# NVIDIA/KAI-Scheduler

Measured on AMD Instinct MI355X. Metric: pod placements/sec (allocate action, synthetic snapshot), higher is better.
Workload: dtype f64

## Files before the change

kai-scheduler_amd/csrc/kai_fill_levels.hpp:

```cpp
#pragma once
#include "kai_fill_counts.hpp"

namespace kai {

constexpr int KFL_LMAX = 8;
constexpr int KFL_RING = 4096;
constexpr int KFL_XR = 32;
constexpr int KFL_SHORT = 16;
constexpr int KFL_JOB_SHIFT = 23;
constexpr int KFL_PAIRS = KFL_LMAX * (KFL_LMAX - 1) / 2;
constexpr int KFL_WKINDS = 7;
KW_BODY uint64_t kfl_cmd(int g, int g2, int k, int per, int tbase) { return (uint64_t)((uint32_t)g | ((uint32_t)g2 << 4) | ((uint32_t)per << 8) | ((uint32_t)k << 12)) | ((uint64_t)(uint32_t)tbase << 32); }
struct FlMove { uint64_t mask; int32_t w; int32_t seq; };
struct FlLds {
    uint64_t ring[KFL_RING];
    uint64_t dummy[64];
    FlMove x[KFL_PAIRS + 1][KFL_XR];
    FlMove xdummy[64];
    int32_t xtail[KFL_PAIRS];
    int32_t cnt0[KBK_GMAX];
    int32_t tail[KFL_LMAX + 1];
    int32_t head, done, fin, b_dec;
    int64_t w_idle[KFL_LMAX + 1], w_total[KFL_LMAX + 1];
#ifdef KFL_PROF
    int64_t wk_cyc[KFL_LMAX][KFL_WKINDS], wk_cnt[KFL_LMAX][KFL_WKINDS];
#endif
};
#if defined(KFL_PROF) && defined(__HIPCC__)
__device__ int64_t kfl_prof_workers[KFL_LMAX][KFL_WKINDS + 1][2];
#endif
KW_BODY int kfl_pair(int g, int g2) { return (g - 1) * (g - 2) / 2 + (g2 - 1); }
KW_BODY int kfl_div(int a, int b) {
    const uint64_t inv = b <= 4 ? 0x2000'2AAB'4000'8000ull : 0x1000'124A'1556'199Aull;
    return (int)(((uint32_t)a * (uint32_t)((inv >> (16 * ((b - 1) & 3))) & 0xffff)) >> 15);
}
KW_BODY uint64_t kfl_read(KW_LDS_PTR(uint64_t) p) { return kw::bcast(*p, 0); }
KW_BODY void kfl_write(KW_LDS_PTR(uint64_t) p, uint64_t v, KW_LDS_PTR(uint64_t) dummy) { KW_LDS_PTR(uint64_t) q = kw::lane() == 0 ? p : dummy + kw::lane(); *q = v; }
KW_BODY int kfl_load(const int32_t* p) { return kw::uni(kw::lds_load_acq(p)); }
struct FlStretch { int flag, first, nt, q; bool valid, is_def; uint64_t defm, todo; };
KW_BODY uint32_t kfl_tab(int lane, int LV) { uint32_t t = 0; for (int g = 1; g <= LV; g++) t |= (uint32_t)(g / (lane + 1)) << (4 * (g - 1)); return t; }
KW_BODY int kfl_quot(uint32_t tab, int g) { return g >= 1 ? (int)((tab >> (4 * (g - 1))) & 15u) : 0; }
KW_BODY void kfl_classify(FlStretch& s, int ucls, int qk, int capq) {
    int q = kw::shfl(qk, ucls >= 0 ? ucls : 0);
    if (ucls < 0 || q > 31) q = ucls < 0 ? 0 : 31;
    const int cap = kw::shfl(capq, q >= 1 ? q - 1 : 63);
    s.q = q;
    s.is_def = s.valid && s.flag == BF_DEAD && q >= 1 && cap < s.nt;
    s.defm = kw::ballot(s.is_def);
    s.todo = kw::ballot(s.valid && s.flag != BF_GATE && !s.is_def);
}

template <int SP>
KW_BODY void kb_fill_levels_t(const KaiCtx& c, RoundParams rp, BucketParams bp) {
    if (kb_round_off(c.bt)) return;
    KW_SHARED FlLds L;
    const BatchCtx& b = c.bt;
    const int tid = kw::tid(), T = kw::bdim(), lane = kw::lane(), C = c.C;
    BkView v; v.NW = bp.nw; v.NW1 = bp.nw1; v.LV = bp.levels;
    unsigned char* dyn = kw::dyn_lds();
    v.gw = (KW_LDS_PTR(uint64_t))dyn; v.s1 = v.gw + (size_t)v.LV * v.NW; v.ok = v.s1 + (size_t)v.LV * v.NW1 + KBK_GMAX;
    const int64_t tstart = kw::clock();
    if (tid < KBK_GMAX) L.cnt0[tid] = 0;
    if (tid <= KFL_LMAX) { L.tail[tid] = 0; L.w_idle[tid] = 0; L.w_total[tid] = 0; }
    if (tid < KFL_PAIRS) L.xtail[tid] = 0;
#ifdef KFL_PROF
    if (tid < KFL_LMAX * KFL_WKINDS) { L.wk_cyc[tid / KFL_WKINDS][tid % KFL_WKINDS] = 0; L.wk_cnt[tid / KFL_WKINDS][tid % KFL_WKINDS] = 0; }
#endif
    for (int i = tid; i < (KFL_PAIRS + 1) * KFL_XR; i += T) L.x[i / KFL_XR][i % KFL_XR].seq = 0;
    if (tid == 0) { L.head = 0; L.done = 0; L.fin = 0; L.b_dec = 0; }
    for (int i = tid; i < v.LV * v.NW; i += T) v.gw[i] = b.bk_words[i];
    kw::sync();
    for (int i = tid; i < v.LV * v.NW1; i += T) {
        const int l = i / v.NW1, w1 = i % v.NW1; uint64_t m = 0; int pop = 0;
        for (int j = 0; j < 64 && w1 * 64 + j < v.NW; j++) { const uint64_t x = v.gw[l * v.NW + w1 * 64 + j]; if (x) { m |= 1ull << j; pop += __builtin_popcountll(x); } }
        v.s1[i] = m;
        if (pop) kw::atomic_add((int32_t*)&L.cnt0[l], pop);
    }
    kw::sync();
    const int V = rp.mode != 1 ? b.q_valid[c.Q] : 0;
    const int wave = kw::uni(tid >> 6);
    if (wave == 0) {
#ifdef KFL_PRIO
        kw::set_prio<KFL_PRIO>();
#endif
        int cnt = lane < v.LV ? L.cnt0[lane] : 0;
        const bool act = lane < C;
        const int qk = act ? (int)c.cls[lane].req[KAI_RES_GPU] : 0x7fffffff;
        const uint32_t tab = kfl_tab(lane, v.LV);
        const int invq = (int)(((lane < 4 ? 0x2000'2AAB'4000'8000ull : 0x1000'124A'1556'199Aull) >> (16 * (lane & 3))) & 0xffff);
        uint32_t nz = (uint32_t)kw::ballot(cnt > 0);
        int decisions = 0, attempted = 0, committed = 0, rollbacks = 0, ops = 0, n_done = rp.start, mismatch = 0;
        int wp = 0, tail_seen = 0, pub = 0, n_mark = 0;
        int64_t a_wait = 0;
#ifdef KFL_PROF
        int64_t pc[5] = {0, 0, 0, 0, 0}; int64_t pt = kw::clock();
        #define KFL_T(i) do { const int64_t n_ = kw::clock(); pc[i] += n_ - pt; pt = n_; } while (0)
#else
        #define KFL_T(i) (void)0
#endif
        auto tails_min = [&]() { int t = lane <= v.LV ? kw::lds_load_acq(&L.tail[lane < v.LV ? lane : KFL_LMAX]) : 0x7fffffff; for (int l = 1; l <= v.LV; l++) { const int o = kw::bcast(t, l); t = o < t ? o : t; } return kw::bcast(t, 0); };
        #define KFL_LEVEL_FOR(qc) ((nz >> ((qc) - 1)) ? (SP ? 32 - __builtin_clz(nz) : (qc) + __builtin_ctz(nz >> ((qc) - 1))) : 0)
        #define KFL_ROOM(n) do { if (wp - tail_seen > KFL_RING - (n)) { kw::lds_store_rel(&L.head, wp); pub = wp; const int64_t w0 = kw::clock(); while (wp - tail_seen > KFL_RING - (n)) { tail_seen = tails_min(); if (wp - tail_seen > KFL_RING - (n)) kw::relax(); } a_wait += kw::clock() - w0; } } while (0)
        #define KFL_EMIT(g_, g2_, k_, per_, tb_) do { KW_LDS_PTR(uint64_t) sl_ = lane == 0 ? (KW_LDS_PTR(uint64_t))&L.ring[wp & (KFL_RING - 1)] : (KW_LDS_PTR(uint64_t))&L.dummy[lane]; *sl_ = kfl_cmd(g_, g2_, k_, per_, tb_) | jbits; wp++; } while (0)
        #define KFL_EVENT(g_, g2_, k_, cg_) do { const int e_g = (g_), e_g2 = (g2_), e_k = (k_), e_cg = (cg_); \
            cnt = kw::writelane(cnt, e_cg - e_k, (e_g - 1) & 63); \
            const uint32_t e_in = e_g2 >= 1 ? 1u << ((e_g2 - 1) & 31) : 0u, e_out = (uint32_t)(e_cg - e_k - 1) >> 31;   \
            cnt = kw::writelane(cnt, kw::bcast(cnt, (e_g2 - 1) & 63) + e_k, (e_g2 - 1) & 63); \
            nz = (nz & ~(e_out << ((e_g - 1) & 31))) | e_in; } while (0)
        #define KFL_STEP(S, EMIT) \
            const uint32_t lv##S = nz >> (qc - 1); \
            ok = kw::nonzero01(lv##S);   \
            const int g##S = lv##S ? (SP ? 32 - __builtin_clz(nz) : qc + __builtin_ctz(lv##S)) : 0, gm1##S = g##S - 1; \
            int r##S = SP ? 1 : (int)((tq >> ((4 * g##S - 4) & 31)) & 15u); r##S = r##S > 1 ? r##S : 1;   \
            const int rem##S = nt - placed; \
            const int kq##S = SP ? rem##S : (int)(((uint32_t)rem##S * (uint32_t)kw::bcast(invq, r##S - 1)) >> 15);   \
            const int cg##S = kw::bcast(cnt, gm1##S & 63); \
            int k##S = kq##S < cg##S ? kq##S : cg##S; k##S = (k##S > 1 ? k##S : 1) * ok;   \
            const int per##S = r##S < rem##S ? r##S : rem##S, g2##S = g##S - per##S * qc; \
            EMIT(g##S, g2##S, k##S, per##S); \
            KFL_EVENT(g##S, g2##S, k##S, cg##S); \
            placed += k##S * per##S
        #define KFL_EMIT_RING(g_, g2_, k_, per_) KFL_EMIT(g_, g2_, k_, per_, first + placed)
        #define KFL_LOW(g_, g2_, k_, per_) (int)((uint32_t)(g_) | ((uint32_t)(g2_) << 4) | ((uint32_t)(per_) << 8) | ((uint32_t)(k_) << 12))
        #define KFL_HOLD0(g_, g2_, k_, per_) c0 = kw::writelane(c0, KFL_LOW(g_, g2_, k_, per_), jj)
        #define KFL_HOLD1(g_, g2_, k_, per_) c1 = kw::writelane(c1, KFL_LOW(g_, g2_, k_, per_), jj)
        #define KFL_GANG_END() \
            okm |= (uint64_t)(uint32_t)(1 - fail) << jj; failm |= (uint64_t)(uint32_t)fail << jj; \
            extra += placed & (0 - fail); \
            cnt = fail ? cnt_s : cnt; nz = fail ? nz_s : nz; wp = fail ? wp_s : wp; \
            const int mism = (int)((uint32_t)(flag - 1) >> 31) ^ fail ^ 1;   \
            mismatch |= mism; last_jj = jj
        int nx_flag = 0, nx_first = 0, nx_nt = 0, nx_ucls = 0;
        if (V > rp.start) { const int gc = rp.start + lane < V ? rp.start + lane : V - 1; nx_flag = b.g_flag[gc]; nx_first = b.g_first[gc]; nx_nt = b.g_nt[gc]; nx_ucls = b.g_ucls[gc]; }
        for (int base = rp.start; base < V && !mismatch; base += 64) {
            const int gi = base + lane;
            FlStretch s; s.valid = gi < V;
            s.flag = s.valid ? nx_flag : (int)BF_GATE; s.first = s.valid ? nx_first : 0; s.nt = s.valid ? nx_nt : 0;
            const int my_ucls = s.valid ? nx_ucls : 0;
            { const int gc = gi + 64 < V ? gi + 64 : V - 1; nx_flag = b.g_flag[gc]; nx_first = b.g_first[gc]; nx_nt = b.g_nt[gc]; nx_ucls = b.g_ucls[gc]; }
            const int jn = V - base < 64 ? V - base : 64;
            int capq = 0;
            for (int g = 1; g <= v.LV; g++) capq += kfl_quot(tab, g) * kw::bcast(cnt, g - 1);
            kfl_classify(s, my_ucls, qk, capq);
            const int my_pack = s.flag | (s.q << 2) | (s.nt << 7) | ((s.q == 0 || s.nt > KFL_SHORT || s.nt < 1) ? 1 << 18 : 0) | (s.flag == BF_OK ? 1 << 19 : 0);
            const uint32_t my_tq = kw::shfl(tab, s.q >= 1 ? s.q - 1 : 63);
            uint64_t longm = kw::ballot(((my_pack >> 18) & 1) != 0);
            uint64_t todo = s.todo, okm = 0, failm = 0, okw = 0;
            int n_out = jn, last_jj = 0, extra = 0;
            attempted += jn; n_done = base + jn;
            KFL_ROOM(1);
#if defined(__HIP_DEVICE_COMPILE__)
            asm volatile("s_waitcnt lgkmcnt(0)" :: "v"(my_tq), "v"(my_pack) : "memory");
#endif
            { KW_LDS_PTR(uint64_t) sl_ = lane == 0 ? (KW_LDS_PTR(uint64_t))&L.ring[wp & (KFL_RING - 1)] : (KW_LDS_PTR(uint64_t))&L.dummy[lane]; *sl_ = 0; wp++; n_mark++; }
            KFL_T(0);
            while (todo) {
                const uint64_t lm = todo & longm;
                const uint64_t below = lm ? (lm & (0 - lm)) - 1 : ~0ull;
                uint64_t hot = todo & below;
                todo &= ~below;
                if (hot) {
                    const uint64_t run0 = hot; uint64_t twor = 0, rest = 0;
                    int c0 = 0, c1 = 0, jj, pred, ok;
                    do {
                        jj = __builtin_ctzll(hot); hot &= hot - 1;
                        const int pack = kw::bcast(my_pack, jj);
                        const uint32_t tq = kw::bcast(my_tq, jj);
                        const int qc = (pack >> 2) & 31, nt = (pack >> 7) & 0x7ff;
                        pred = (pack >> 19) & 1;
                        KFL_T(1);
                        const uint32_t nz_s = nz;
                        int placed = 0;
                        KFL_STEP(A, KFL_HOLD0);
                        if (__builtin_expect(placed < nt * ok, 0)) {
                            int cnt_s = kw::writelane(cnt, kw::bcast(cnt, (g2A - 1) & 63) - kA, (g2A - 1) & 63); cnt_s = kw::writelane(cnt_s, cgA, gm1A & 63);
                            KFL_STEP(B, KFL_HOLD1);
                            if (!ok) { cnt = cnt_s; nz = nz_s; extra += placed; }
                            else if (placed < nt) {
                                cnt = cnt_s; nz = nz_s; longm |= 1ull << jj; rest = hot | (1ull << jj); hot = 0; ok = pred;
                            } else twor |= 1ull << jj;
                        }
                        KFL_T(2);
                        okw |= (uint64_t)(uint32_t)ok << jj;
                        hot = kw::opaque(pred == ok ? hot : (uint64_t)0);
                        KFL_T(3);
                    } while (hot);
                    mismatch |= pred ^ ok;
                    const uint64_t walked = run0 & ((2ull << jj) - 1) & ~rest, okr = walked & okw;
                    failm |= walked & ~okw; hot |= rest;
                    okm |= okr;
                    if (mismatch) last_jj = 63 - __builtin_clzll(walked);
                    if (okr) {
                        const int n_my = (int)((okr >> lane) & 1ull) + (int)((twor >> lane) & 1ull);
                        const int incl = kw::wave_scan_add(n_my), n_run = kw::bcast(incl, 63);
                        KFL_ROOM(n_run);
                        const int pos = wp + incl - n_my;
                        const uint32_t jb = (uint32_t)lane << KFL_JOB_SHIFT;
                        if (n_my >= 1) L.ring[pos & (KFL_RING - 1)] = (uint64_t)((uint32_t)c0 | jb) | ((uint64_t)(uint32_t)s.first << 32);
                        if (n_my >= 2) L.ring[(pos + 1) & (KFL_RING - 1)] = (uint64_t)((uint32_t)c1 | jb) | ((uint64_t)(uint32_t)(s.first + ((c0 >> 12) & 0x7ff) * ((c0 >> 8) & 15)) << 32);
                        wp += n_run;
                        kw::lds_store_rel(&L.head, wp); pub = wp;
                    }
                    KFL_T(3);
                }
                todo |= hot;
                if (mismatch) break;
                if (!hot && lm) {
                    const int jj = __builtin_ctzll(todo); todo &= todo - 1;
                    const int pack = kw::bcast(my_pack, jj), first = kw::bcast(s.first, jj);
                    const uint32_t tq = kw::bcast(my_tq, jj);
                    const int flag = pack & 3, qc = (pack >> 2) & 31, nt = (pack >> 7) & 0x7ff;
                    const uint64_t jbits = (uint64_t)((uint32_t)jj << KFL_JOB_SHIFT);
                    KFL_T(1);
                    const int cnt_s = cnt, wp_s = wp; const uint32_t nz_s = nz;
                    int placed = 0, ok = 1;
                    KFL_ROOM(nt);
                    if (!qc) {
                        for (int tb = 0; tb < nt && ok; tb += 64) {
                            const int my_cls = tb + lane < nt ? b.t_cls[first + tb + lane] : 0;
                            const int tc = nt - tb < 64 ? nt - tb : 64;
                            for (int ti = 0; ti < tc; ti++) {
                                const int q1 = kw::bcast(qk, kw::bcast(my_cls, ti));
                                const int g = q1 <= 31 ? KFL_LEVEL_FOR(q1) : 0;
                                if (!g) { ok = 0; break; }
                                KFL_EMIT(g, g - q1, 1, 1, first + placed);
                                KFL_EVENT(g, g - q1, 1, kw::bcast(cnt, g - 1));
                                placed++;
                            }
                        }
                    } else while ((placed < nt) & (ok != 0)) { KFL_STEP(L, KFL_EMIT_RING); }
                    const int fail = ok ^ 1;
                    KFL_T(2);
                    KFL_GANG_END();
                    if (wp - pub >= 64) { kw::lds_store_rel(&L.head, wp); pub = wp; }
                    KFL_T(3);
                    if (mism) break;
                }
            }
            if (mismatch) { n_done = base + last_jj + 1; n_out = last_jj + 1; attempted -= jn - n_out; }
            KFL_T(3);
            {
                const uint64_t outm = n_out >= 64 ? ~0ull : (1ull << n_out) - 1;
                const int nfail = __builtin_popcountll(s.defm & outm) + __builtin_popcountll(failm);
                decisions += nfail + extra; rollbacks += 2 * nfail;
                const bool my_ok = (okm >> lane) & 1ull;
                const int myv = my_ok ? s.nt : 0, incl = kw::wave_scan_add(myv);
                const int my_stmt = committed + rp.stmt0 + __builtin_popcountll(okm & ((1ull << lane) - 1)), my_opoff = ops + rp.ops0 + incl - myv;
                if (lane < n_out) { b.g_out[base + lane] = (uint8_t)(my_ok ? BF_OK : BF_DEAD); b.g_opoff[base + lane] = my_opoff; b.g_stmt[base + lane] = my_stmt; }
                committed += __builtin_popcountll(okm); ops += kw::bcast(incl, 63); decisions += kw::bcast(incl, 63);
            }
            if (wp != pub) { kw::lds_store_rel(&L.head, wp); pub = wp; }
            KFL_T(4);
        }
        #undef KFL_LEVEL_FOR
        #undef KFL_ROOM
        #undef KFL_EMIT
        #undef KFL_EVENT
        #undef KFL_STEP
        #undef KFL_EMIT_RING
        #undef KFL_LOW
        #undef KFL_HOLD0
        #undef KFL_HOLD1
        #undef KFL_GANG_END
        if (lane == 0) L.fin = n_done;
        kw::lds_store_rel(&L.head, wp);
        kw::lds_store_rel(&L.done, 1);
        const uint64_t dead = kw::ballot(act && (qk > 32 || (nz >> (qk - 1)) == 0));
        if (lane == 0) {
            FillStatus s; s.n_done = n_done; s.mismatch = mismatch; s.all_dead = (C > 0 && dead == (C >= 64 ? ~0ull : ((1ull << C) - 1))) ? 1 : 0; s.planned = V; s.floor_stop = 0; s.pad = 0;
            s.decisions = decisions; s.attempted = attempted; s.committed = committed; s.rollbacks = rollbacks; s.ops = ops; s.dead_mask = dead;
            s.cycles_total = kw::clock() - tstart; s.cycles_load = a_wait; s.cycles_update = 0; s.cycles_rescan = 0; s.block_loads = 0;
            s.rescans1 = 0; s.rescans2 = wp - n_mark; s.rescans3 = 0;
#ifdef KFL_PROF
            s.cycles_load = pc[0]; s.cycles_update = pc[1]; s.cycles_rescan = pc[2]; s.block_loads = pc[3]; s.rescans1 = pc[4];
#endif
            b.fs[0] = s; b.dead_mask[0] = dead;
        }
    } else if (wave <= v.LV) {
        const int G = wave, lw = (G - 1) * v.NW, l1 = (G - 1) * v.NW1;
        KW_LDS_PTR(uint64_t) dm = (KW_LDS_PTR(uint64_t))&L.dummy[0];
        uint64_t s1v = lane < v.NW1 ? v.s1[l1 + lane] : 0;
        uint64_t s2 = kw::ballot(s1v != 0);
        int firstn = KB_INF, cw = -1; uint64_t curw = 0;
        auto refill = [&]() { if (!s2) { firstn = KB_INF; cw = -1; curw = 0; return; } const int w1 = __builtin_ctzll(s2); cw = w1 * 64 + __builtin_ctzll(kw::bcast(s1v, w1)); curw = kfl_read(&v.gw[lw + cw]); firstn = (cw << 6) + __builtin_ctzll(curw); };
        refill();
        int xp = 0, xseen = 0, xc = 0;
        int tail = 0; int64_t w_idle = 0; const int64_t w_start = kw::clock();
#ifdef KFL_PROF
        int64_t wt = kw::clock();
        #define KFL_WT0() (wt = kw::clock())
        #define KFL_WK(kind_) do { const int64_t n_ = kw::clock(); if (lane == 0) { L.wk_cyc[G - 1][kind_] += n_ - wt; L.wk_cnt[G - 1][kind_]++; } wt = n_; } while (0)
#else
        #define KFL_WT0() (void)0
        #define KFL_WK(kind_) (void)0
#endif
        for (;;) {
            const int head = kfl_load(&L.head);
            if (tail == head) {
                if (kfl_load(&L.done) && tail == kfl_load(&L.head)) break;
                const int64_t i0 = kw::clock(); while (kfl_load(&L.head) == tail && !kfl_load(&L.done)) kw::relax(); w_idle += kw::clock() - i0;
                continue;
            }
            while (tail < head) {
                const int nb = head - tail < 64 ? head - tail : 64;
                const uint64_t mc = L.ring[(tail + lane) & (KFL_RING - 1)];
                uint64_t mine = kw::ballot(lane < nb && ((int)(mc & 15) == G || (int)((mc >> 4) & 15) == G));
                while (mine) {
                    KFL_WT0();
                    const int ci = __builtin_ctzll(mine); mine &= mine - 1;
                    const int ca = kw::bcast((int)(uint32_t)mc, ci);
                    const int g = ca & 15, g2 = (ca >> 4) & 15;
                    if (g == G) {
                        const int per = (ca >> 8) & 15; int left = (ca >> 12) & 0x7ff, tb = kw::bcast((int)(uint32_t)(mc >> 32), ci);
                        const int pr = g2 >= 1 ? kfl_pair(G, g2) : KFL_PAIRS;
                        const int xl = (g2 - 1) & 63;
#ifdef KFL_PROF
                        const int k_all = left; int n_words = 0, n_emptied = 0;
#endif
                        if (__builtin_expect(left == 1, 1)) {
                            const int w = cw; const uint64_t mask = curw & (0 - curw), neww = curw ^ mask;
                            b.t_node[tb + (lane < per ? lane : per - 1)] = firstn;
                            kfl_write(&v.gw[lw + w], neww, dm);
                            const int n_w = kw::bcast(xp, xl);
                            if (__builtin_expect(n_w - kw::bcast(xseen, xl) >= KFL_XR, 0)) { int t; while (n_w - (t = kfl_load(&L.xtail[pr])) >= KFL_XR) kw::relax(); if (lane == xl) xseen = t; }
                            KW_LDS_PTR(FlMove) e = lane == 0 ? (KW_LDS_PTR(FlMove))&L.x[pr][n_w & (KFL_XR - 1)] : (KW_LDS_PTR(FlMove))&L.xdummy[lane];
                            e->mask = mask; e->w = w | (1 << 30);
                            kw::lds_store_ordered((int32_t*)&e->seq, n_w + 1);
                            xp += lane == g2 - 1 ? 1 : 0;
                            if (__builtin_expect(neww != 0, 1)) { curw = neww; firstn = (w << 6) + __builtin_ctzll(neww); }
                            else {
                                const int w1 = w >> 6; const uint64_t m1 = kw::bcast(s1v, w1) & ~(1ull << (w & 63));
                                s1v = kw::writelane(s1v, m1, w1);
                                s2 &= ~((uint64_t)(uint32_t)(1 - kw::nonzero01((uint32_t)m1 | (uint32_t)(m1 >> 32))) << w1);
                                refill();
#ifdef KFL_PROF
                                n_emptied++;
#endif
                            }
                            left = 0;
                        }
                        while (__builtin_expect(left > 0, 0)) {
                            const int w = cw; const uint64_t word = curw;
                            const int pop = __builtin_popcountll(word), m = left < pop ? left : pop;
                            const int r = kw::rank_below(word);
                            const bool sel = ((word >> lane) & 1ull) != 0 && r < m;
                            const uint64_t mask = kw::ballot(sel), neww = word ^ mask;
                            const int one = m == 1, lastn = (w << 6) + 63 - __builtin_clzll(mask);
                            const int val = sel ? (w << 6) + lane : lastn;
                            const int onem = 0 - one, off1 = lane < per ? lane : per - 1, offm = sel ? r * per : m * per - 1;
                            int a = tb + ((off1 & onem) | (offm & ~onem));
                            b.t_node[a] = val;
                            if (__builtin_expect((per & ~onem) > 1, 0)) {
                                const int stp = sel ? 1 : 0;
                                _Pragma("nounroll") for (int j = 1; j < per; j++) { a += stp; b.t_node[a] = val; }
                            }
                            kfl_write(&v.gw[lw + w], neww, dm);
                            left -= m; tb += m * per;
                            const int n_w = kw::bcast(xp, xl);
                            if (__builtin_expect(n_w - kw::bcast(xseen, xl) >= KFL_XR, 0)) { int t; while (n_w - (t = kfl_load(&L.xtail[pr])) >= KFL_XR) kw::relax(); if (lane == xl) xseen = t; }
                            KW_LDS_PTR(FlMove) e = lane == 0 ? (KW_LDS_PTR(FlMove))&L.x[pr][n_w & (KFL_XR - 1)] : (KW_LDS_PTR(FlMove))&L.xdummy[lane];
                            e->mask = mask; e->w = w | (left == 0 ? 1 << 30 : 0);
                            kw::lds_store_ordered((int32_t*)&e->seq, n_w + 1);
                            xp += lane == g2 - 1 ? 1 : 0;
                            if (__builtin_expect(neww != 0, 1)) { curw = neww; firstn = (w << 6) + __builtin_ctzll(neww); }
                            else {
                                const int w1 = w >> 6; const uint64_t m1 = kw::bcast(s1v, w1) & ~(1ull << (w & 63));
                                s1v = kw::writelane(s1v, m1, w1);
                                s2 &= ~((uint64_t)(uint32_t)(1 - kw::nonzero01((uint32_t)m1 | (uint32_t)(m1 >> 32))) << w1);
                                refill();
#ifdef KFL_PROF
                                n_emptied++;
#endif
                            }
#ifdef KFL_PROF
                            n_words++;
#endif
                        }
#ifdef KFL_PROF
                        if (k_all == 1) { if (n_emptied) KFL_WK(1); else KFL_WK(0); } else if (n_words == 1) KFL_WK(2); else KFL_WK(3);
#endif
                    } else {
                        const int pr = kfl_pair(g, G);
                        for (bool last = false; !last;) {
                            const int n_r = kw::bcast(xc, g - 1);
                            const int sl = n_r & (KFL_XR - 1);
                            int sq = kw::lds_load_ordered(&L.x[pr][sl].seq), wf_v = kw::lds_load_relaxed(&L.x[pr][sl].w); uint64_t mk_v = kw::lds_load_relaxed(&L.x[pr][sl].mask);
                            if (__builtin_expect(kw::uni(sq) != n_r + 1, 0)) { const int64_t i0 = kw::clock(); while (kfl_load(&L.x[pr][sl].seq) != n_r + 1) kw::relax(); w_idle += kw::clock() - i0; wf_v = kw::lds_load_relaxed(&L.x[pr][sl].w); mk_v = kw::lds_load_relaxed(&L.x[pr][sl].mask); KFL_WT0(); }
                            const int wf = kw::bcast(wf_v, 0), w = wf & 0x3fffffff; const uint64_t mask = kw::bcast(mk_v, 0);
                            last = (wf >> 30) & 1;
                            kw::lds_store_ordered(&L.xtail[pr], n_r + 1);
                            if (lane == g - 1) xc++;
                            if (w == cw) { curw |= mask; kfl_write(&v.gw[lw + w], curw, dm); firstn = (w << 6) + __builtin_ctzll(curw); KFL_WK(4); }
                            else {
                                const int w1 = w >> 6;
#ifdef KFL_PROF
                                const bool was_empty = ((kw::bcast(s1v, w1) >> (w & 63)) & 1ull) == 0;
#endif
                                { KW_LDS_PTR(uint64_t) q = lane == 0 ? (KW_LDS_PTR(uint64_t))&v.gw[lw + w] : dm + lane; kw::lds_or(q, mask); }
                                s1v = kw::writelane(s1v, kw::bcast(s1v, w1) | (1ull << (w & 63)), w1); s2 |= 1ull << w1;
                                const int n = (w << 6) + __builtin_ctzll(mask), fn = kw::uni(firstn);
                                const bool lower = n < fn;
                                firstn = lower ? n : fn; cw = lower ? w : cw; curw = lower ? mask : curw;
#ifdef KFL_PROF
                                if (was_empty) KFL_WK(5); else KFL_WK(6);
#endif
                            }
                        }
                    }
                }
                tail += nb;
            }
            kw::lds_store_rel(&L.tail[G - 1], tail);
        }
        #undef KFL_WT0
        #undef KFL_WK
        if (lane == 0) { L.w_idle[G - 1] = w_idle; L.w_total[G - 1] = kw::clock() - w_start; }
    } else if (wave == v.LV + 1) {
        const int qk = lane < C ? (int)c.cls[lane].req[KAI_RES_GPU] : 0x7fffffff;
        const uint32_t tab = kfl_tab(lane, v.LV);
        int capq = 0;
// ... 70 lines not shown
```

kai-scheduler_amd/csrc/kai_simt.hpp:

```cpp
#pragma once
#include <stdint.h>

#if defined(__HIPCC__)
#include <hip/hip_runtime.h>

#include "kai_wave.hpp"
#define KW_DEV __device__ __forceinline__
#define KW_BODY __device__ __forceinline__
#define KW_SHARED __shared__
#define KW_LDS_PTR(T) T __attribute__((address_space(3)))*
namespace kw {
KW_DEV int tid() { return (int)threadIdx.x; }
KW_DEV int bid() { return (int)blockIdx.x; }
KW_DEV int bdim() { return (int)blockDim.x; }
KW_DEV int gdim() { return (int)gridDim.x; }
KW_DEV int lane() { return (int)(threadIdx.x & 63); }
KW_DEV void sync() { __syncthreads(); }
KW_DEV uint64_t ballot(bool p) { return (uint64_t)__ballot(p); }
template <class T> KW_DEV T shfl(T v, int src) { return __shfl(v, src, 64); }
KW_DEV uint64_t shfl(uint64_t v, int src) { return (uint64_t)__shfl((unsigned long long)v, src, 64); }
KW_DEV int64_t shfl(int64_t v, int src) { return (int64_t)__shfl((long long)v, src, 64); }
template <class T> KW_DEV T shfl_up(T v, int d) { return __shfl_up(v, d, 64); }
KW_DEV uint64_t wave_max_u64(uint64_t v) { return (uint64_t)kai::wave_max_u64((unsigned long long)v); }
KW_DEV int bcast(int v, int src) { return __builtin_amdgcn_readlane(v, __builtin_amdgcn_readfirstlane(src)); }
KW_DEV uint32_t bcast(uint32_t v, int src) { return (uint32_t)bcast((int)v, src); }
KW_DEV uint64_t bcast(uint64_t v, int src) { const int s = __builtin_amdgcn_readfirstlane(src); return ((uint64_t)(uint32_t)__builtin_amdgcn_readlane((int)(v >> 32), s) << 32) | (uint32_t)__builtin_amdgcn_readlane((int)v, s); }
KW_DEV double bcast(double v, int src) { return __longlong_as_double((long long)bcast((uint64_t)__double_as_longlong(v), src)); }
KW_DEV int uni(int v) { return __builtin_amdgcn_readfirstlane(v); }
KW_DEV uint32_t uni(uint32_t v) { return (uint32_t)__builtin_amdgcn_readfirstlane((int)v); }
KW_DEV uint64_t uni(uint64_t v) { return ((uint64_t)(uint32_t)__builtin_amdgcn_readfirstlane((int)(v >> 32)) << 32) | (uint32_t)__builtin_amdgcn_readfirstlane((int)v); }
extern "C" __device__ int kw_llvm_writelane(int v, int dst, int old) __asm("llvm.amdgcn.writelane.i32");
KW_DEV int writelane(int old, int v, int dst) { return kw_llvm_writelane(__builtin_amdgcn_readfirstlane(v), __builtin_amdgcn_readfirstlane(dst), old); }
KW_DEV uint64_t writelane(uint64_t old, uint64_t v, int dst) { return ((uint64_t)(uint32_t)writelane((int)(old >> 32), (int)(v >> 32), dst) << 32) | (uint32_t)writelane((int)old, (int)v, dst); }
KW_DEV int rank_below(uint64_t m) { return (int)__builtin_amdgcn_mbcnt_hi((uint32_t)(m >> 32), __builtin_amdgcn_mbcnt_lo((uint32_t)m, 0u)); }
KW_DEV int nonzero01(uint32_t v) { int r; asm("s_min_u32 %0, %1, 1" : "=s"(r) : "s"(v) : "scc"); return r; }
KW_DEV uint64_t opaque(uint64_t v) { v = uni(v); asm("" : "+s"(v)); return v; }
template <int P> KW_DEV void set_prio() { __builtin_amdgcn_s_setprio(P); }
KW_DEV int atomic_add(int32_t* p, int v) { return atomicAdd(p, v); }
KW_DEV int atomic_min(int32_t* p, int v) { return atomicMin(p, v); }
KW_DEV int atomic_max(int32_t* p, int v) { return atomicMax(p, v); }
KW_DEV unsigned long long atomic_add(unsigned long long* p, unsigned long long v) { return atomicAdd(p, v); }
KW_DEV unsigned long long atomic_or(unsigned long long* p, unsigned long long v) { return atomicOr(p, v); }
KW_DEV double atomic_add(double* p, double v) { return atomicAdd(p, v); }
KW_DEV uint32_t atomic_or32(uint32_t* p, uint32_t v) { return atomicOr(p, v); }
KW_DEV int64_t clock() { return (int64_t)clock64(); }
KW_DEV unsigned char* dyn_lds() { extern __shared__ __align__(16) unsigned char kw_dyn_lds_[]; return kw_dyn_lds_; }
KW_DEV void fence() { __threadfence(); }
KW_DEV void wave_sync() { __builtin_amdgcn_fence(__ATOMIC_RELEASE, "workgroup"); __builtin_amdgcn_wave_barrier(); __builtin_amdgcn_fence(__ATOMIC_ACQUIRE, "workgroup"); }
KW_DEV void lds_order() { __builtin_amdgcn_fence(__ATOMIC_RELEASE, "wavefront"); __builtin_amdgcn_wave_barrier(); __builtin_amdgcn_fence(__ATOMIC_ACQUIRE, "wavefront"); }
KW_DEV uint64_t lds_xor(KW_LDS_PTR(uint64_t) p, uint64_t v) { return __hip_atomic_fetch_xor(p, v, __ATOMIC_RELAXED, __HIP_MEMORY_SCOPE_WAVEFRONT); }
KW_DEV void lds_or(KW_LDS_PTR(uint64_t) p, uint64_t v) { (void)__hip_atomic_fetch_or(p, v, __ATOMIC_RELAXED, __HIP_MEMORY_SCOPE_WAVEFRONT); }
KW_DEV void expect_uniform(long long) {}
KW_DEV void fence_wg() { __builtin_amdgcn_fence(__ATOMIC_RELEASE, "workgroup"); __builtin_amdgcn_fence(__ATOMIC_ACQUIRE, "workgroup"); }
KW_DEV int lds_load_acq(const int32_t* p) { return __hip_atomic_load(p, __ATOMIC_ACQUIRE, __HIP_MEMORY_SCOPE_WORKGROUP); }
KW_DEV void lds_store_rel(int32_t* p, int v) { __hip_atomic_store(p, v, __ATOMIC_RELEASE, __HIP_MEMORY_SCOPE_WORKGROUP); }
KW_DEV void relax() { __builtin_amdgcn_s_sleep(1); }
KW_DEV void lds_store_ordered(int32_t* p, int v) { __builtin_amdgcn_fence(__ATOMIC_RELEASE, "wavefront"); __hip_atomic_store(p, v, __ATOMIC_RELAXED, __HIP_MEMORY_SCOPE_WORKGROUP); }
KW_DEV int lds_load_ordered(const int32_t* p) { const int v = __hip_atomic_load(p, __ATOMIC_RELAXED, __HIP_MEMORY_SCOPE_WORKGROUP); __builtin_amdgcn_fence(__ATOMIC_ACQUIRE, "wavefront"); return v; }
KW_DEV int lds_load_relaxed(const int32_t* p) { return __hip_atomic_load(p, __ATOMIC_RELAXED, __HIP_MEMORY_SCOPE_WORKGROUP); }
KW_DEV uint64_t lds_load_relaxed(const uint64_t* p) { return __hip_atomic_load(p, __ATOMIC_RELAXED, __HIP_MEMORY_SCOPE_WORKGROUP); }
}

#else
#include <cstdio>
#include <cstdlib>
#include <cstring>
#include <functional>
#include <vector>
#define KW_DEV inline
#define KW_BODY inline
#define KW_LDS_PTR(T) T*
#define KW_SHARED static
namespace kw {

extern "C" void kw_switch_ctx(void** save_sp, void* load_sp);
#if defined(__x86_64__)
asm(R"(
.text
.globl kw_switch_ctx
.type kw_switch_ctx,@function
kw_switch_ctx:
    pushq %rbp
    pushq %rbx
    pushq %r12
    pushq %r13
    pushq %r14
    pushq %r15
    movq %rsp, (%rdi)
    movq %rsi, %rsp
    popq %r15
    popq %r14
    popq %r13
    popq %r12
    popq %rbx
    popq %rbp
    ret
.size kw_switch_ctx,.-kw_switch_ctx
)");
#else
#error "the host emulator's context switch is written for x86-64"
#endif

enum FiberState : int { F_RUN = 0, F_WAIT_BLOCK = 1, F_WAIT_WAVE = 2, F_DONE = 3 };
struct Fiber { void* sp = nullptr; int state = F_DONE; char* stack = nullptr; int line = 0; };
struct Emu {
    std::vector<Fiber> fibers; std::vector<char*> stacks;
    void* sched_sp = nullptr;
    int cur = -1, block = 0, bdim = 0, gdim = 0;
    const std::function<void()>* body = nullptr;
    uint64_t xchg[64 * 64];
    std::vector<unsigned char> lds;
    static constexpr size_t STACK = 128 * 1024;
};
inline Emu& emu() { static Emu e; return e; }
inline void fiber_yield() { Emu& e = emu(); kw_switch_ctx(&e.fibers[e.cur].sp, e.sched_sp); }
inline void fiber_entry() {
    Emu& e = emu();
    (*e.body)();
    e.fibers[e.cur].state = F_DONE;
    fiber_yield();
    std::abort();
}
inline void launch(int grid, int block, size_t dyn_lds_bytes, const std::function<void()>& body) {
    Emu& e = emu();
    if (grid <= 0 || block <= 0) return;
    if (block > 64 * 64) { std::fprintf(stderr, "kw::launch: workgroup too large\n"); std::abort(); }
    e.lds.assign(dyn_lds_bytes + 64, 0);
    e.body = &body; e.bdim = block; e.gdim = grid;
    if ((int)e.fibers.size() < block) e.fibers.resize(block);
    while ((int)e.stacks.size() < block) e.stacks.push_back(static_cast<char*>(std::malloc(Emu::STACK)));
    for (int b = 0; b < grid; b++) {
        e.block = b;
        for (int t = 0; t < block; t++) {
            Fiber& f = e.fibers[t]; f.stack = e.stacks[t]; f.state = F_RUN;
            uintptr_t top = (reinterpret_cast<uintptr_t>(f.stack) + Emu::STACK) & ~uintptr_t(15);
            void** sp = reinterpret_cast<void**>(top) - 2;
            *sp = reinterpret_cast<void*>(&fiber_entry);
            for (int i = 0; i < 6; i++) *--sp = nullptr;
            f.sp = sp;
        }
        int live = block;
        static const int order = [] { const char* v = std::getenv("KW_EMU_ORDER"); return v ? std::atoi(v) : 0; }();
        static uint64_t rng = [] { const char* v = std::getenv("KW_EMU_SEED"); return 0x9e3779b97f4a7c15ull + (v ? (uint64_t)std::atoll(v) * 0x100000001b3ull : 0); }();
        while (live > 0) {
            bool progress = false;
            const int nwv = (block + 63) / 64;
            for (int wi = 0; wi < nwv; wi++) {
                const int w = order == 1 ? nwv - 1 - wi : wi;
                if (order == 2) { rng = rng * 6364136223846793005ull + 1442695040888963407ull; if ((rng >> 40) & 1) continue; }
                for (int t = w * 64; t < block && t < w * 64 + 64; t++) {
                    if (e.fibers[t].state != F_RUN) continue;
                    e.cur = t; kw_switch_ctx(&e.sched_sp, e.fibers[t].sp);
                    progress = true;
                    if (e.fibers[t].state == F_DONE) live--;
                }
            }
            if (order == 2 && !progress) { bool any = false; for (int t = 0; t < block; t++) if (e.fibers[t].state == F_RUN) any = true; if (any) continue; }
            bool all_block = true; int waiting = 0;
            for (int t = 0; t < block; t++) { int s = e.fibers[t].state; if (s == F_RUN || s == F_WAIT_WAVE) all_block = false; if (s == F_WAIT_BLOCK) waiting++; }
            if (all_block && waiting) { for (int t = 0; t < block; t++) if (e.fibers[t].state == F_WAIT_BLOCK) e.fibers[t].state = F_RUN; progress = true; }
            for (int w = 0; w * 64 < block; w++) {
                bool all = true; int nw = 0;
                for (int t = w * 64; t < block && t < w * 64 + 64; t++) { int s = e.fibers[t].state; if (s == F_RUN || s == F_WAIT_BLOCK) all = false; if (s == F_WAIT_WAVE) nw++; }
                if (all && nw) { for (int t = w * 64; t < block && t < w * 64 + 64; t++) if (e.fibers[t].state == F_WAIT_WAVE) e.fibers[t].state = F_RUN; progress = true; }
            }
            if (!progress && live > 0) {
                std::fprintf(stderr, "kw::launch: deadlock (a collective not reached by every live lane); block %d, lanes parked at source lines:", b);
                for (int t = 0; t < block && t < 64; t++) std::fprintf(stderr, " %d:%s%d", t, e.fibers[t].state == F_WAIT_BLOCK ? "B" : e.fibers[t].state == F_WAIT_WAVE ? "W" : e.fibers[t].state == F_DONE ? "done" : "run", e.fibers[t].line);
                std::fprintf(stderr, "\n"); std::abort();
            }
        }
    }
    e.body = nullptr;
}
inline int tid() { return emu().cur; }
inline int bid() { return emu().block; }
inline int bdim() { return emu().bdim; }
inline int gdim() { return emu().gdim; }
inline int lane() { return emu().cur & 63; }
inline void sync(int line = __builtin_LINE()) { Emu& e = emu(); e.fibers[e.cur].line = line; e.fibers[e.cur].state = F_WAIT_BLOCK; fiber_yield(); }
inline void wave_bar(int line = 0) { Emu& e = emu(); if (line) e.fibers[e.cur].line = line; e.fibers[e.cur].state = F_WAIT_WAVE; fiber_yield(); }
inline uint64_t* wave_slots() { Emu& e = emu(); return e.xchg + (size_t)(e.cur >> 6) * 64; }
inline bool lane_live(int l) { Emu& e = emu(); int t = (e.cur & ~63) + l; return t < e.bdim && e.fibers[t].state != F_DONE; }
template <class T> inline T shfl(T v, int src, int line = __builtin_LINE()) {
    static_assert(sizeof(T) <= 8, "shfl: 8 bytes at most");
    uint64_t raw = 0; std::memcpy(&raw, &v, sizeof(T));
    wave_slots()[lane()] = raw; wave_bar(line);
    uint64_t got = wave_slots()[src & 63]; wave_bar();
    T r; std::memcpy(&r, &got, sizeof(T)); return r;
}
template <class T> inline T shfl_up(T v, int d) { int l = lane(); T r = shfl(v, l >= d ? l - d : l); return l >= d ? r : v; }
inline uint64_t ballot(bool p, int line = __builtin_LINE()) {
    wave_slots()[lane()] = p ? 1 : 0; wave_bar(line);
    uint64_t m = 0; for (int l = 0; l < 64; l++) if (lane_live(l) && wave_slots()[l]) m |= 1ull << l;
    wave_bar(); return m;
}
inline uint64_t wave_max_u64(uint64_t v, int line = __builtin_LINE()) {
    wave_slots()[lane()] = v; wave_bar(line);
    uint64_t m = 0; for (int l = 0; l < 64; l++) if (lane_live(l) && wave_slots()[l] > m) m = wave_slots()[l];
    wave_bar(); return m;
}
template <class T> inline T bcast(T v, int src, int line = __builtin_LINE()) { return shfl(v, src, line); }
template <class T> inline T uni(T v) { return v; }
inline int writelane(int old, int v, int dst) { return lane() == dst ? v : old; }
inline uint64_t writelane(uint64_t old, uint64_t v, int dst) { return lane() == dst ? v : old; }
inline int rank_below(uint64_t m) { return __builtin_popcountll(m & ((1ull << lane()) - 1)); }
inline int nonzero01(uint32_t v) { return v ? 1 : 0; }
inline uint64_t opaque(uint64_t v) { return v; }
template <int P> inline void set_prio() {}
inline int atomic_add(int32_t* p, int v) { int o = *p; *p = o + v; return o; }
inline int atomic_min(int32_t* p, int v) { int o = *p; if (v < o) *p = v; return o; }
inline int atomic_max(int32_t* p, int v) { int o = *p; if (v > o) *p = v; return o; }
inline unsigned long long atomic_add(unsigned long long* p, unsigned long long v) { unsigned long long o = *p; *p = o + v; return o; }
inline unsigned long long atomic_or(unsigned long long* p, unsigned long long v) { unsigned long long o = *p; *p = o | v; return o; }
inline double atomic_add(double* p, double v) { double o = *p; *p = o + v; return o; }
inline uint32_t atomic_or32(uint32_t* p, uint32_t v) { uint32_t o = *p; *p = o | v; return o; }
inline int64_t clock() { return 0; }
inline unsigned char* dyn_lds() { Emu& e = emu(); return reinterpret_cast<unsigned char*>((reinterpret_cast<uintptr_t>(e.lds.data()) + 15) & ~uintptr_t(15)); }
inline void fence() {}
inline void fence_wg() {}
inline int lds_load_acq(const int32_t* p) { return *p; }
inline void lds_store_rel(int32_t* p, int v) { *p = v; }
inline void lds_store_ordered(int32_t* p, int v) { *p = v; }
inline int lds_load_ordered(const int32_t* p) { return *p; }
inline int lds_load_relaxed(const int32_t* p) { return *p; }
inline uint64_t lds_load_relaxed(const uint64_t* p) { return *p; }
inline void relax(int line = __builtin_LINE()) { wave_bar(line); }
inline void wave_sync(int line = __builtin_LINE()) { wave_bar(line); }
inline void lds_order(int line = __builtin_LINE()) { wave_bar(line); }
inline uint64_t lds_xor(uint64_t* p, uint64_t v) { const uint64_t o = *p; *p = o ^ v; return o; }
inline void lds_or(uint64_t* p, uint64_t v) { *p |= v; }
inline void expect_uniform(long long v, int line = __builtin_LINE()) { const long long v0 = shfl(v, 0, line); if (v != v0) { std::fprintf(stderr, "kw: value not uniform at line %d: lane %d has %lld, lane 0 has %lld\n", line, lane(), v, v0); std::abort(); } }
}
#endif

namespace kw {
KW_DEV void wave_argmax_first(uint64_t& key, int& n) {
    const uint64_t m = wave_max_u64(key);
    const uint64_t win = ballot(key == m);
    const int l = __builtin_ctzll(win);
    n = shfl(n, l);
    key = m;
}
template <class T> KW_DEV T wave_scan_add(T v) {
    for (int d = 1; d < 64; d <<= 1) { T o = shfl_up(v, d); if (lane() >= d) v = v + o; }
    return v;
}
#if defined(__HIPCC__)
#define KW_DPP_MOV(x, ctrl, rmask) __builtin_amdgcn_update_dpp(0, (int)(x), ctrl, rmask, 0xf, false)
template <> KW_DEV int wave_scan_add<int>(int v) {
    v += KW_DPP_MOV(v, 0x111, 0xf); v += KW_DPP_MOV(v, 0x112, 0xf); v += KW_DPP_MOV(v, 0x114, 0xf); v += KW_DPP_MOV(v, 0x118, 0xf);
    v += KW_DPP_MOV(v, 0x142, 0xa); v += KW_DPP_MOV(v, 0x143, 0xc);
    return v;
}
template <int CTRL, int RMASK> KW_DEV int dpp_mov32(int x) { return __builtin_amdgcn_update_dpp(0, x, CTRL, RMASK, 0xf, false); }
template <int CTRL, int RMASK> KW_DEV uint64_t dpp_mov64(uint64_t x) { return ((uint64_t)(unsigned)dpp_mov32<CTRL, RMASK>((int)(x >> 32)) << 32) | (unsigned)dpp_mov32<CTRL, RMASK>((int)x); }
template <> KW_DEV double wave_scan_add<double>(double v) {
#define KW_DPP_ADD_F64(ctrl, rmask) { const long long b_ = __double_as_longlong(v); const unsigned lo_ = (unsigned)KW_DPP_MOV((unsigned)b_, ctrl, rmask), hi_ = (unsigned)KW_DPP_MOV((unsigned)((unsigned long long)b_ >> 32), ctrl, rmask); v = v + __longlong_as_double((long long)(((unsigned long long)hi_ << 32) | lo_)); }
    KW_DPP_ADD_F64(0x111, 0xf) KW_DPP_ADD_F64(0x112, 0xf) KW_DPP_ADD_F64(0x114, 0xf) KW_DPP_ADD_F64(0x118, 0xf) KW_DPP_ADD_F64(0x142, 0xa) KW_DPP_ADD_F64(0x143, 0xc)
#undef KW_DPP_ADD_F64
    return v;
}
#endif
}
```

Before: 8.229 million.

## Precompute per-lane fill decisions in a table and shift level indexing by one

The hot gang-placement loop now uses a per-lane decision word computed in parallel across the wave (KFL_TABLE) while the level bitmap is unchanged. It replaces the serial per-gang KFL_STEP computation with a broadcast and a few scalar ops, and recomputes the table only when the bitmap changes. Level counts are re-indexed from 1 with bit 0 of nz used as a sentinel, so level 0 absorbs gangs that drain a level. Bit updates use scalar s_bitset instructions. This adds complexity and recomputation whenever nz changes, and carries a correctness risk in the reworked mismatch and fail bookkeeping.

```diff
diff --git a/kai-scheduler_amd/csrc/kai_fill_levels.hpp b/kai-scheduler_amd/csrc/kai_fill_levels.hpp
--- a/kai-scheduler_amd/csrc/kai_fill_levels.hpp
+++ b/kai-scheduler_amd/csrc/kai_fill_levels.hpp
@@ -83,12 +83,12 @@
 #ifdef KFL_PRIO
         kw::set_prio<KFL_PRIO>();
 #endif
-        int cnt = lane < v.LV ? L.cnt0[lane] : 0;
+        int cnt = lane >= 1 && lane <= v.LV ? L.cnt0[lane - 1] : 0;
         const bool act = lane < C;
         const int qk = act ? (int)c.cls[lane].req[KAI_RES_GPU] : 0x7fffffff;
         const uint32_t tab = kfl_tab(lane, v.LV);
         const int invq = (int)(((lane < 4 ? 0x2000'2AAB'4000'8000ull : 0x1000'124A'1556'199Aull) >> (16 * (lane & 3))) & 0xffff);
-        uint32_t nz = (uint32_t)kw::ballot(cnt > 0);
+        uint32_t nz = (uint32_t)kw::ballot(cnt > 0) | 1u;
         int decisions = 0, attempted = 0, committed = 0, rollbacks = 0, ops = 0, n_done = rp.start, mismatch = 0;
         int wp = 0, tail_seen = 0, pub = 0, n_mark = 0;
         int64_t a_wait = 0;
@@ -99,22 +99,22 @@
         #define KFL_T(i) (void)0
 #endif
         auto tails_min = [&]() { int t = lane <= v.LV ? kw::lds_load_acq(&L.tail[lane < v.LV ? lane : KFL_LMAX]) : 0x7fffffff; for (int l = 1; l <= v.LV; l++) { const int o = kw::bcast(t, l); t = o < t ? o : t; } return kw::bcast(t, 0); };
-        #define KFL_LEVEL_FOR(qc) ((nz >> ((qc) - 1)) ? (SP ? 32 - __builtin_clz(nz) : (qc) + __builtin_ctz(nz >> ((qc) - 1))) : 0)
+        #define KFL_LEVEL_FOR(qc) (((nz >> 1) >> ((qc) - 1)) ? (SP ? 31 - __builtin_clz(nz) : (qc) + __builtin_ctz((nz >> 1) >> ((qc) - 1))) : 0)
         #define KFL_ROOM(n) do { if (wp - tail_seen > KFL_RING - (n)) { kw::lds_store_rel(&L.head, wp); pub = wp; const int64_t w0 = kw::clock(); while (wp - tail_seen > KFL_RING - (n)) { tail_seen = tails_min(); if (wp - tail_seen > KFL_RING - (n)) kw::relax(); } a_wait += kw::clock() - w0; } } while (0)
         #define KFL_EMIT(g_, g2_, k_, per_, tb_) do { KW_LDS_PTR(uint64_t) sl_ = lane == 0 ? (KW_LDS_PTR(uint64_t))&L.ring[wp & (KFL_RING - 1)] : (KW_LDS_PTR(uint64_t))&L.dummy[lane]; *sl_ = kfl_cmd(g_, g2_, k_, per_, tb_) | jbits; wp++; } while (0)
-        #define KFL_EVENT(g_, g2_, k_, cg_) do { const int e_g = (g_), e_g2 = (g2_), e_k = (k_), e_cg = (cg_); \
-            cnt = kw::writelane(cnt, e_cg - e_k, (e_g - 1) & 63); \
-            const uint32_t e_in = e_g2 >= 1 ? 1u << ((e_g2 - 1) & 31) : 0u, e_out = (uint32_t)(e_cg - e_k - 1) >> 31;   \
-            cnt = kw::writelane(cnt, kw::bcast(cnt, (e_g2 - 1) & 63) + e_k, (e_g2 - 1) & 63); \
-            nz = (nz & ~(e_out << ((e_g - 1) & 31))) | e_in; } while (0)
+        #define KFL_EVENT(g_, g2_, k_, cg_) do { const int e_g = (g_), e_g2 = (g2_) > 0 ? (g2_) : 0, e_k = (k_), e_cg = (cg_); \
+            const int e_t = kw::bcast(cnt, e_g2 & 63); \
+            cnt = kw::writelane(cnt, e_cg - e_k, e_g & 63); \
+            cnt = kw::writelane(cnt, e_t + e_k, e_g2 & 63);   \
+            nz = kw::bit_set(kw::bit_clear(nz, e_cg == e_k ? e_g : 31), e_g2); } while (0)
         #define KFL_STEP(S, EMIT) \
-            const uint32_t lv##S = nz >> (qc - 1); \
+            const uint32_t lv##S = nz >> qc; \
             ok = kw::nonzero01(lv##S);   \
-            const int g##S = lv##S ? (SP ? 32 - __builtin_clz(nz) : qc + __builtin_ctz(lv##S)) : 0, gm1##S = g##S - 1; \
+            const int g##S = lv##S ? (SP ? 31 - __builtin_clz(nz) : qc + __builtin_ctz(lv##S)) : 0; \
             int r##S = SP ? 1 : (int)((tq >> ((4 * g##S - 4) & 31)) & 15u); r##S = r##S > 1 ? r##S : 1;   \
             const int rem##S = nt - placed; \
             const int kq##S = SP ? rem##S : (int)(((uint32_t)rem##S * (uint32_t)kw::bcast(invq, r##S - 1)) >> 15);   \
-            const int cg##S = kw::bcast(cnt, gm1##S & 63); \
+            const int cg##S = kw::bcast(cnt, g##S & 63); \
             int k##S = kq##S < cg##S ? kq##S : cg##S; k##S = (k##S > 1 ? k##S : 1) * ok;   \
             const int per##S = r##S < rem##S ? r##S : rem##S, g2##S = g##S - per##S * qc; \
             EMIT(g##S, g2##S, k##S, per##S); \
@@ -122,15 +122,26 @@
             placed += k##S * per##S
         #define KFL_EMIT_RING(g_, g2_, k_, per_) KFL_EMIT(g_, g2_, k_, per_, first + placed)
         #define KFL_LOW(g_, g2_, k_, per_) (int)((uint32_t)(g_) | ((uint32_t)(g2_) << 4) | ((uint32_t)(per_) << 8) | ((uint32_t)(k_) << 12))
-        #define KFL_HOLD0(g_, g2_, k_, per_) c0 = kw::writelane(c0, KFL_LOW(g_, g2_, k_, per_), jj)
         #define KFL_HOLD1(g_, g2_, k_, per_) c1 = kw::writelane(c1, KFL_LOW(g_, g2_, k_, per_), jj)
+        #define KFL_TABLE() do { \
+            const int t_q = s.q >= 1 ? s.q : 1, t_nt = s.nt; \
+            const uint32_t t_lv = nz >> t_q; \
+            const int t_g = SP ? 31 - __builtin_clz(nz) : t_q + __builtin_ctz(t_lv | 0x80000000u); \
+            int t_r = SP ? 1 : (int)((my_tq >> ((4 * t_g - 4) & 31)) & 15u); t_r = t_r > 1 ? t_r : 1; \
+            const int t_kq = SP ? t_nt : kfl_div(t_nt, t_r), t_kq1 = t_kq > 1 ? t_kq : 1; \
+            const int t_per = t_r < t_nt ? t_r : t_nt, t_g2 = t_g - t_per * t_q; \
+            const uint32_t t_p = s.flag == BF_OK ? 1u : 0u; \
+            const uint32_t t_w = (uint32_t)t_g | ((uint32_t)t_g2 << 4) | ((uint32_t)t_per << 8) | ((uint32_t)t_kq1 << 23) | (t_kq1 * t_per < t_nt ? 1u << 28 : 0u) | (1u << 29) | ((t_p ^ 1u) << 30); \
+            dw = t_lv ? t_w : t_p << 30; nz_tab = nz; mism = kw::ballot(((dw >> 30) & 1u) != 0); } while (0)
+        #define KFL_CUT(h) do { const uint64_t c_m = (h) & mism, c_keep = c_m ? ((c_m & (0 - c_m)) << 1) - 1 : ~0ull; held = (h) & ~c_keep; (h) &= c_keep; } while (0)
         #define KFL_GANG_END() \
             okm |= (uint64_t)(uint32_t)(1 - fail) << jj; failm |= (uint64_t)(uint32_t)fail << jj; \
             extra += placed & (0 - fail); \
             cnt = fail ? cnt_s : cnt; nz = fail ? nz_s : nz; wp = fail ? wp_s : wp; \
-            const int mism = (int)((uint32_t)(flag - 1) >> 31) ^ fail ^ 1;   \
-            mismatch |= mism; last_jj = jj
+            const int g_mis = (int)((uint32_t)(flag - 1) >> 31) ^ fail ^ 1;   \
+            mismatch |= g_mis; last_jj = jj
         int nx_flag = 0, nx_first = 0, nx_nt = 0, nx_ucls = 0;
+        uint32_t dw = 0, nz_tab = ~0u; uint64_t mism = 0;
         if (V > rp.start) { const int gc = rp.start + lane < V ? rp.start + lane : V - 1; nx_flag = b.g_flag[gc]; nx_first = b.g_first[gc]; nx_nt = b.g_nt[gc]; nx_ucls = b.g_ucls[gc]; }
         for (int base = rp.start; base < V && !mismatch; base += 64) {
             const int gi = base + lane;
@@ -140,12 +151,13 @@
             { const int gc = gi + 64 < V ? gi + 64 : V - 1; nx_flag = b.g_flag[gc]; nx_first = b.g_first[gc]; nx_nt = b.g_nt[gc]; nx_ucls = b.g_ucls[gc]; }
             const int jn = V - base < 64 ? V - base : 64;
             int capq = 0;
-            for (int g = 1; g <= v.LV; g++) capq += kfl_quot(tab, g) * kw::bcast(cnt, g - 1);
+            for (int g = 1; g <= v.LV; g++) capq += kfl_quot(tab, g) * kw::bcast(cnt, g);
             kfl_classify(s, my_ucls, qk, capq);
             const int my_pack = s.flag | (s.q << 2) | (s.nt << 7) | ((s.q == 0 || s.nt > KFL_SHORT || s.nt < 1) ? 1 << 18 : 0) | (s.flag == BF_OK ? 1 << 19 : 0);
             const uint32_t my_tq = kw::shfl(tab, s.q >= 1 ? s.q - 1 : 63);
             uint64_t longm = kw::ballot(((my_pack >> 18) & 1) != 0);
-            uint64_t todo = s.todo, okm = 0, failm = 0, okw = 0;
+            nz_tab = ~0u;
+            uint64_t todo = s.todo, okm = 0, failm = 0;
             int n_out = jn, last_jj = 0, extra = 0;
             attempted += jn; n_done = base + jn;
             KFL_ROOM(1);
@@ -160,32 +172,46 @@
                 uint64_t hot = todo & below;
                 todo &= ~below;
                 if (hot) {
-                    const uint64_t run0 = hot; uint64_t twor = 0, rest = 0;
-                    int c0 = 0, c1 = 0, jj, pred, ok;
+                    const uint64_t run0 = hot; uint64_t twor = 0, rest = 0, fail2 = 0, held;
+                    int c0 = 0, c1 = 0, jj; uint32_t w;
+                    if (nz != nz_tab) { KFL_TABLE(); }
+                    KFL_CUT(hot);
                     do {
-                        jj = __builtin_ctzll(hot); hot &= hot - 1;
-                        const int pack = kw::bcast(my_pack, jj);
-                        const uint32_t tq = kw::bcast(my_tq, jj);
-                        const int qc = (pack >> 2) & 31, nt = (pack >> 7) & 0x7ff;
-                        pred = (pack >> 19) & 1;
+                        jj = __builtin_ctzll(hot); hot = kw::bit_clear(hot, jj);
+                        w = kw::bcast(dw, jj);
                         KFL_T(1);
-                        const uint32_t nz_s = nz;
-                        int placed = 0;
-                        KFL_STEP(A, KFL_HOLD0);
-                        if (__builtin_expect(placed < nt * ok, 0)) {
-                            int cnt_s = kw::writelane(cnt, kw::bcast(cnt, (g2A - 1) & 63) - kA, (g2A - 1) & 63); cnt_s = kw::writelane(cnt_s, cgA, gm1A & 63);
-                            KFL_STEP(B, KFL_HOLD1);
-                            if (!ok) { cnt = cnt_s; nz = nz_s; extra += placed; }
-                            else if (placed < nt) {
-                                cnt = cnt_s; nz = nz_s; longm |= 1ull << jj; rest = hot | (1ull << jj); hot = 0; ok = pred;
-                            } else twor |= 1ull << jj;
+                        const int g = w & 15, g2 = (w >> 4) & 15;
+                        const int cg = kw::bcast(cnt, g), t2 = kw::bcast(cnt, g2);
+                        const int kq = (w >> 23) & 31, k = kq < cg ? kq : cg;
+                        c0 = kw::writelane(c0, (int)(w | ((uint32_t)k << 12)), jj);
+                        cnt = kw::writelane(cnt, cg - k, g);
+                        cnt = kw::writelane(cnt, t2 + k, g2);
+                        nz = kw::bit_set(kw::bit_clear(nz, cg == k ? g : 31), g2);
+                        if (__builtin_expect(kw::opaque((uint32_t)(k ^ (int)((w >> 23) & 63)) | (nz ^ nz_tab)) != 0, 0)) {
+                            if (k != (int)((w >> 23) & 63)) {
+                                const int pack = kw::bcast(my_pack, jj);
+                                const uint32_t tq = kw::bcast(my_tq, jj);
+                                const int qc = (pack >> 2) & 31, nt = (pack >> 7) & 0x7ff, pred = (pack >> 19) & 1;
+                                const uint32_t nz_s = nz_tab;
+                                int placed = k * (int)((w >> 8) & 15), ok;
+                                int cnt_s = kw::writelane(cnt, t2, g2); cnt_s = kw::writelane(cnt_s, cg, g);
+                                KFL_STEP(B, KFL_HOLD1);
+                                if (!ok) { cnt = cnt_s; nz = nz_s; extra += placed; fail2 |= 1ull << jj; }
+                                else if (placed < nt) {
+                                    cnt = cnt_s; nz = nz_s; longm |= 1ull << jj; rest = hot | held | (1ull << jj); hot = 0; held = 0; ok = pred;
+                                } else twor |= 1ull << jj;
+                                w = (w & ~(1u << 30)) | ((uint32_t)(pred ^ ok) << 30);
+                            }
+                            if ((w >> 30) & 1) { hot = 0; held = 0; }
+                            else {
+                                if (nz != nz_tab) { KFL_TABLE(); }
+                                hot |= held; KFL_CUT(hot);
+                            }
                         }
                         KFL_T(2);
-                        okw |= (uint64_t)(uint32_t)ok << jj;
-                        hot = kw::opaque(pred == ok ? hot : (uint64_t)0);
-                        KFL_T(3);
                     } while (hot);
-                    mismatch |= pred ^ ok;
+                    mismatch |= (int)((w >> 30) & 1);
+                    const uint64_t okw = kw::ballot(((c0 >> 29) & 1) != 0) & ~fail2;
                     const uint64_t walked = run0 & ((2ull << jj) - 1) & ~rest, okr = walked & okw;
                     failm |= walked & ~okw; hot |= rest;
                     okm |= okr;
@@ -196,7 +222,7 @@
                         KFL_ROOM(n_run);
                         const int pos = wp + incl - n_my;
                         const uint32_t jb = (uint32_t)lane << KFL_JOB_SHIFT;
-                        if (n_my >= 1) L.ring[pos & (KFL_RING - 1)] = (uint64_t)((uint32_t)c0 | jb) | ((uint64_t)(uint32_t)s.first << 32);
+                        if (n_my >= 1) L.ring[pos & (KFL_RING - 1)] = (uint64_t)(((uint32_t)c0 & 0x7fffffu) | jb) | ((uint64_t)(uint32_t)s.first << 32);
                         if (n_my >= 2) L.ring[(pos + 1) & (KFL_RING - 1)] = (uint64_t)((uint32_t)c1 | jb) | ((uint64_t)(uint32_t)(s.first + ((c0 >> 12) & 0x7ff) * ((c0 >> 8) & 15)) << 32);
                         wp += n_run;
                         kw::lds_store_rel(&L.head, wp); pub = wp;
@@ -224,7 +250,7 @@
                                 const int g = q1 <= 31 ? KFL_LEVEL_FOR(q1) : 0;
                                 if (!g) { ok = 0; break; }
                                 KFL_EMIT(g, g - q1, 1, 1, first + placed);
-                                KFL_EVENT(g, g - q1, 1, kw::bcast(cnt, g - 1));
+                                KFL_EVENT(g, g - q1, 1, kw::bcast(cnt, g));
                                 placed++;
                             }
                         }
@@ -234,7 +260,7 @@
                     KFL_GANG_END();
                     if (wp - pub >= 64) { kw::lds_store_rel(&L.head, wp); pub = wp; }
                     KFL_T(3);
-                    if (mism) break;
+                    if (g_mis) break;
                 }
             }
             if (mismatch) { n_done = base + last_jj + 1; n_out = last_jj + 1; attempted -= jn - n_out; }
@@ -259,13 +285,14 @@
         #undef KFL_STEP
         #undef KFL_EMIT_RING
         #undef KFL_LOW
-        #undef KFL_HOLD0
+        #undef KFL_TABLE
+        #undef KFL_CUT
         #undef KFL_HOLD1
         #undef KFL_GANG_END
         if (lane == 0) L.fin = n_done;
         kw::lds_store_rel(&L.head, wp);
         kw::lds_store_rel(&L.done, 1);
-        const uint64_t dead = kw::ballot(act && (qk > 32 || (nz >> (qk - 1)) == 0));
+        const uint64_t dead = kw::ballot(act && (qk > 32 || ((nz >> 1) >> (qk - 1)) == 0));
         if (lane == 0) {
             FillStatus s; s.n_done = n_done; s.mismatch = mismatch; s.all_dead = (C > 0 && dead == (C >= 64 ? ~0ull : ((1ull << C) - 1))) ? 1 : 0; s.planned = V; s.floor_stop = 0; s.pad = 0;
             s.decisions = decisions; s.attempted = attempted; s.committed = committed; s.rollbacks = rollbacks; s.ops = ops; s.dead_mask = dead;
diff --git a/kai-scheduler_amd/csrc/kai_simt.hpp b/kai-scheduler_amd/csrc/kai_simt.hpp
--- a/kai-scheduler_amd/csrc/kai_simt.hpp
+++ b/kai-scheduler_amd/csrc/kai_simt.hpp
@@ -34,7 +34,11 @@
 KW_DEV uint64_t writelane(uint64_t old, uint64_t v, int dst) { return ((uint64_t)(uint32_t)writelane((int)(old >> 32), (int)(v >> 32), dst) << 32) | (uint32_t)writelane((int)old, (int)v, dst); }
 KW_DEV int rank_below(uint64_t m) { return (int)__builtin_amdgcn_mbcnt_hi((uint32_t)(m >> 32), __builtin_amdgcn_mbcnt_lo((uint32_t)m, 0u)); }
 KW_DEV int nonzero01(uint32_t v) { int r; asm("s_min_u32 %0, %1, 1" : "=s"(r) : "s"(v) : "scc"); return r; }
+KW_DEV uint32_t bit_clear(uint32_t v, int bit) { asm("s_bitset0_b32 %0, %1" : "+s"(v) : "s"(bit)); return v; }
+KW_DEV uint32_t bit_set(uint32_t v, int bit) { asm("s_bitset1_b32 %0, %1" : "+s"(v) : "s"(bit)); return v; }
+KW_DEV uint64_t bit_clear(uint64_t v, int bit) { asm("s_bitset0_b64 %0, %1" : "+s"(v) : "s"(bit)); return v; }
 KW_DEV uint64_t opaque(uint64_t v) { v = uni(v); asm("" : "+s"(v)); return v; }
+KW_DEV uint32_t opaque(uint32_t v) { v = uni(v); asm("" : "+s"(v)); return v; }
 template <int P> KW_DEV void set_prio() { __builtin_amdgcn_s_setprio(P); }
 KW_DEV int atomic_add(int32_t* p, int v) { return atomicAdd(p, v); }
 KW_DEV int atomic_min(int32_t* p, int v) { return atomicMin(p, v); }
@@ -206,7 +210,11 @@
 inline uint64_t writelane(uint64_t old, uint64_t v, int dst) { return lane() == dst ? v : old; }
 inline int rank_below(uint64_t m) { return __builtin_popcountll(m & ((1ull << lane()) - 1)); }
 inline int nonzero01(uint32_t v) { return v ? 1 : 0; }
+inline uint32_t bit_clear(uint32_t v, int bit) { return v & ~(1u << (bit & 31)); }
+inline uint32_t bit_set(uint32_t v, int bit) { return v | (1u << (bit & 31)); }
+inline uint64_t bit_clear(uint64_t v, int bit) { return v & ~(1ull << (bit & 63)); }
 inline uint64_t opaque(uint64_t v) { return v; }
+inline uint32_t opaque(uint32_t v) { return v; }
 template <int P> inline void set_prio() {}
 inline int atomic_add(int32_t* p, int v) { int o = *p; *p = o + v; return o; }
 inline int atomic_min(int32_t* p, int v) { int o = *p; if (v < o) *p = v; return o; }
```

Result: faster. 8.490 million (median of 6 runs) (+3.2%).
